# 0xPolygonZero/proof-protocol-decoder

Hardware: NVIDIA B200
Metric: mpt_nodes_keccak_hashed_per_sec (higher is better)
Workload: dtype u64

## Files before the change

### proof_protocol_decoder_b200/csrc/gpu_pre_image.cu

```cuda
#include "host_pipeline.h"

namespace ppd {

bool gpu_parse_enabled() {
#ifdef PPD_HOSTPROF
  return false;
#else
  return getenv("PPD_HOST_PARSE") == nullptr;
#endif
}

struct Carve {
  uint8_t* base;
  size_t off = 0;
  template <class T>
  T* take(size_t count) {
    off = (off + 255) & ~(size_t)255;
    T* r = reinterpret_cast<T*>(base + off);
    off += count * sizeof(T);
    return r;
  }
};

void upload_bytes(Lane* L, Job& J, uint8_t* dst, const uint8_t* src, size_t n) {
// ... 104 lines not shown
  const uint32_t n_ins = hr[PARSE_R_NINS];
  if (n_ins == 0 || n_ins > n) return false;
  if ((uint64_t)n_ins * 4 > (uint64_t)n + 256) return false;
  ParseTree T{};
  T.wit = B.wit, T.n = B.n, T.n_ins = n_ins, T.result = B.result;
  T.cnt_stride = ((size_t)n_ins + 1 + 3) & ~(size_t)3;
  uint32_t* ins_pos = nullptr;
  auto layout_b = [&](Carve& c) {
    const size_t n1 = (size_t)n_ins + 1;
    const size_t n_m1 = (n1 + 63) / 64, n_m2 = (n_m1 + 63) / 64, n_m3 = (n_m2 + 63) / 64;
    ins_pos = c.take<uint32_t>(n_ins);
    T.meta = c.take<uint32_t>(n_ins);
    T.knib = c.take<uint8_t>(n_ins);
    T.delta = c.take<uint32_t>(n1);
    T.hb = c.take<uint32_t>(n1);
    T.h16 = c.take<int16_t>(n1);
    T.m0 = c.take<int16_t>(8 * n_m1);
    T.m1 = c.take<int16_t>(n_m1);
    T.m2 = c.take<int16_t>(n_m2);
    T.m3 = c.take<int16_t>(n_m3);
    T.parent = c.take<uint32_t>(n_ins);
    T.info = c.take<uint32_t>(n_ins);
    T.aux0 = c.take<uint32_t>(n_ins);
    T.keyed = c.take<uint32_t>(n_ins);
    T.pending = c.take<uint32_t>(n_ins);
    T.lvlmax = c.take<uint32_t>(n_ins);
    T.cnt = c.take<uint32_t>(PARSE_N_CNT * T.cnt_stride);
    T.scn = c.take<uint32_t>(PARSE_N_CNT * T.cnt_stride);
    T.scan_tmp = c.take<uint32_t>(parse_scan_tmp_words(n1, PARSE_N_CNT));
  };
  {
    Carve sz{nullptr};
    layout_b(sz);
    L->d_pb.reserve(sz.off + 256);
    Carve c{L->d_pb.as<uint8_t>()};
    layout_b(c);
  }
  T.ins_pos = ins_pos;
  CUDA_OK(cudaEventRecord(L->ev0, st));
  launch_parse_scatter(B, ins_pos, st);
  L->stats.kernel_launches += 1 + launch_parse_tree(T, st);
  CUDA_OK(cudaGetLastError());
  CUDA_OK(cudaEventRecord(L->ev1, st));
  result_to_host();
  lane_sync(L);
  phase_ms();
  lap("p:B");
  trace_mark(L, "parse_b");
  if (hr[PARSE_R_FLAG] != 0 || hr[PARSE_R_HEIGHT] != 1) return false;
// ... 234 lines not shown
```

### proof_protocol_decoder_b200/csrc/ppd_kernels.h

```cpp
#pragma once
#include <cuda_runtime.h>

#include <cstdint>

#include "arena.h"
#include "txn_core.h"

namespace ppd {

void launch_keccak256_batch(const uint8_t* data, const uint64_t* offsets, uint32_t n, uint8_t* out, cudaStream_t st);
void launch_keccak256_ranges(const uint8_t* data, const uint64_t* begin_end, uint32_t n, uint8_t* out, cudaStream_t st);
void launch_hash_level(const ArenaView& A, const uint32_t* order, uint32_t begin, uint32_t end, cudaStream_t st);
static const uint32_t ORDER_MAX_BINS = 4096;
void launch_order_by_level_class(const NodeRec* nodes, const uint16_t* level, uint32_t n, uint32_t n_bins, uint16_t* keys, uint32_t* bins,
                                 uint32_t* order, cudaStream_t st, uint32_t first = 0, const uint32_t* n_dev = nullptr);

struct CopyBatch {
  static const uint32_t MAX = 16;
  void* dst[MAX];
  const void* src[MAX];
  unsigned long long bytes[MAX];
  uint32_t n = 0;
};
void launch_copy_segments(const CopyBatch& B, cudaStream_t st);
// ... 101 lines not shown
  uint32_t* exit1;
  uint16_t* step1;
  uint32_t* exit2;
  uint32_t* group_entry;
  uint32_t* tile_entry;
  uint32_t* bitmap;
  uint32_t* tile_count;
  uint32_t* tile_base;
  uint32_t* scan_tmp;
  uint32_t* result;
};
struct ParseTree {
  const uint8_t* wit;
  uint32_t n, n_ins;
  const uint32_t* ins_pos;
  uint32_t* meta;
  uint8_t* knib;
  uint32_t* delta;
  uint32_t* hb;
  int16_t *h16, *m0, *m1, *m2, *m3;
  uint32_t* parent;
  uint32_t* info;
  uint32_t* aux0;
  uint32_t* keyed;
  uint32_t *pending, *lvlmax;
  uint32_t *cnt, *scn;
  size_t cnt_stride;
  uint32_t* scan_tmp;
  uint32_t* result;
};
struct ParseEmit {
  ParseTree T;
  NodeRec* nodes;
  uint16_t* level;
  uint8_t *key_pool, *val_pool, *hash_pool;
  uint32_t* child_pool;
  AccountRec* accounts;
  uint32_t* acct_list;
  uint64_t* code_se;
  uint32_t* code_list;
  const uint8_t* code_digest;
  uint32_t n_keyed;
};
size_t parse_scan_tmp_words(size_t n, uint32_t K);
uint32_t launch_parse_bounds(const ParseBounds& B, cudaStream_t st);
void launch_parse_scatter(const ParseBounds& B, uint32_t* ins_pos, cudaStream_t st);
uint32_t launch_parse_tree(const ParseTree& T, cudaStream_t st);
void launch_parse_code_list(const ParseEmit& E, cudaStream_t st);
// ... 17 lines not shown
```

### proof_protocol_decoder_b200/csrc/ppd_parse.cu

```cuda
#include <cstdint>

#include "../../include/ppd_flat.h"
#include "../../include/ppd_status.h"
#include "arena.h"
#include "ppd_kernels.h"

namespace ppd {

namespace {

constexpr uint32_t TILE = PARSE_TILE;
constexpr uint32_t PERR = PARSE_ERR;
constexpr uint32_t NONE = 0xffffffffu;
constexpr uint32_t HASH_BASE = 0x80000000u;

__constant__ uint8_t C_EMPTY_TRIE_HASH[32] = {0x56, 0xe8, 0x1f, 0x17, 0x1b, 0xcc, 0x55, 0xa6, 0xff, 0x83, 0x45, 0xe6, 0x92, 0xc0, 0xf8, 0x6e,
                                              0x5b, 0x48, 0xe0, 0x1b, 0x99, 0x6c, 0xad, 0xc0, 0x01, 0x62, 0x2f, 0xb5, 0xe3, 0x63, 0xb4, 0x21};
__constant__ uint8_t C_EMPTY_CODE_HASH[32] = {0xc5, 0xd2, 0x46, 0x01, 0x86, 0xf7, 0x23, 0x3c, 0x92, 0x7e, 0x7d, 0xb2, 0xdc, 0xc7, 0x03, 0xc0,
                                              0xe5, 0x00, 0xb6, 0x53, 0xca, 0x82, 0x27, 0x3b, 0x7b, 0xfa, 0xd8, 0x04, 0x5d, 0x85, 0xa4, 0x70};

struct Ins {
  uint32_t op, next, flags, aux;
  uint32_t key_pos, key_len, val_pos, val_len;
  uint64_t nonce;
};

__device__ __forceinline__ bool cbor_head(const uint8_t* w, uint32_t n, uint32_t& pos, uint32_t& major, uint64_t& arg) {
  if (pos >= n) return false;
  uint32_t b = w[pos++];
  major = b >> 5;
  uint32_t ai = b & 31;
  if (ai < 24) {
    arg = ai;
    return true;
  }
  if (ai > 27) return false;
  uint32_t wd = 1u << (ai - 24);
  if (n - pos < wd) return false;
  arg = 0;
  for (uint32_t i = 0; i < wd; i++) arg = (arg << 8) | w[pos++];
  return true;
// ... 44 lines not shown
        if (!cbor_head(w, n, pos, major, arg) || major != 0) return PPD_ERR_INVALID_BYTES_FOR_TYPE;
        o.nonce = arg;
      }
      if (o.flags & 8) {
        if (!cbor_bytes(w, n, pos, o.val_pos, o.val_len) || o.val_len > 32) return PPD_ERR_INVALID_BYTE_VECTOR;
      }
      if (o.flags & 1) {
        if (!cbor_head(w, n, pos, major, arg) || major != 0) return PPD_ERR_INVALID_BYTES_FOR_TYPE;
      }
      break;
    case PPD_OP_EMPTY_ROOT:
      break;
    default:
      return PPD_ERR_INVALID_OPERATOR;
  }
  o.next = pos;
  return 0;
}
__device__ __forceinline__ uint32_t key_nibble_count(const uint8_t* __restrict__ w, uint32_t at, uint32_t len) {
  if (len == 0) return 0;
  if (len == 1) return 1;
  return 2 * (len - 1) - (__ldg(w + at) & 1u);
}
__device__ __forceinline__ void set_nib(uint8_t* pk, uint32_t d, uint32_t nib) { pk[d >> 1] |= (uint8_t)((d & 1) ? nib : (nib << 4)); }
__device__ __forceinline__ void put_key_nibbles(uint8_t* pk, uint32_t d, const uint8_t* __restrict__ w, uint32_t at, uint32_t len) {
  if (len == 0) return;
  if (len == 1) {
    set_nib(pk, d, __ldg(w + at) & 15u);
    return;
  }
  uint32_t cnt = 2 * (len - 1) - (__ldg(w + at) & 1u);
  for (uint32_t i = 0; i < cnt; i++) {
    uint32_t b = __ldg(w + at + 1 + (i >> 1));
    set_nib(pk, d + i, (i & 1) ? (b & 15u) : (b >> 4));
  }
}
__device__ __forceinline__ uint32_t nth_set_bit(uint32_t mask, uint32_t k) {
  for (uint32_t i = 0; i < k; i++) mask &= mask - 1;
  return mask ? (uint32_t)__ffs(mask) - 1 : 0u;
}

constexpr int TE_THREADS = 512;
constexpr uint32_t HALO = 128;

__device__ __forceinline__ void stage_tile(uint8_t* sb, const uint8_t* __restrict__ w, uint32_t n, uint32_t base, uint32_t tid, uint32_t nthreads) {
  const uint4* src = reinterpret_cast<const uint4*>(w + base);
  uint4* dst = reinterpret_cast<uint4*>(sb);
  const uint32_t avail = ((uint64_t)base + TILE + HALO <= (uint64_t)n + 48) ? (TILE + HALO) / 16 : (n + 48 - base) / 16;
  for (uint32_t k = tid; k < (TILE + HALO) / 16; k += nthreads) dst[k] = k < avail ? __ldg(src + k) : make_uint4(0, 0, 0, 0);
}

constexpr uint32_t TE_SMEM_BYTES = 4 * TILE + 4 * 2 * TILE + (TILE + HALO) + 16;

__global__ void __launch_bounds__(TE_THREADS, 4) tile_exit_kernel(const uint8_t* __restrict__ w, uint32_t n, uint32_t* __restrict__ exit1,
                                                                  uint16_t* __restrict__ step1) {
  extern __shared__ __align__(16) uint8_t te_smem[];
  uint32_t* nxt = reinterpret_cast<uint32_t*>(te_smem);
  uint16_t* step = reinterpret_cast<uint16_t*>(te_smem + 4 * TILE);
  uint16_t* active = step + TILE;
// ... 169 lines not shown
__global__ void __launch_bounds__(TILE / 32) ins_scatter_kernel(const uint32_t* __restrict__ bitmap, const uint32_t* __restrict__ tile_base,
                                                                uint32_t* __restrict__ ins_pos) {
  __shared__ uint32_t wsum[TILE / 32 / 32];
  const uint32_t t = blockIdx.x, tid = threadIdx.x;
  uint32_t word = bitmap[(size_t)t * (TILE / 32) + tid];
  uint32_t c = __popc(word), incl = c;
  for (int off = 1; off < 32; off <<= 1) {
    uint32_t x = __shfl_up_sync(0xffffffffu, incl, off);
    if ((tid & 31) >= (uint32_t)off) incl += x;
  }
  if ((tid & 31) == 31) wsum[tid >> 5] = incl;
  __syncthreads();
  uint32_t before = 0;
  for (uint32_t k = 0; k < (tid >> 5); k++) before += wsum[k];
  uint32_t at = tile_base[t] + before + incl - c;
  const uint32_t p0 = t * TILE + tid * 32;
  while (word) {
    uint32_t b = (uint32_t)__ffs(word) - 1;
    word &= word - 1;
    ins_pos[at++] = p0 + b;
  }
}

constexpr int MS_B = 256, MS_ITEMS = 4, MS_ELEMS = MS_B * MS_ITEMS;

__global__ void __launch_bounds__(MS_B) mscan_block_kernel(const uint32_t* __restrict__ in, uint32_t* __restrict__ out, uint32_t n, size_t stride,
                                                           uint32_t* __restrict__ block_sums, size_t sums_stride) {
  __shared__ uint32_t warp_sums[MS_B / 32];
  const uint32_t k = blockIdx.y;
  in += k * stride, out += k * stride;
  uint32_t base = blockIdx.x * MS_ELEMS + threadIdx.x * MS_ITEMS;
  uint32_t v[MS_ITEMS], sum = 0;
#pragma unroll
  for (int q = 0; q < MS_ITEMS; q++) {
    v[q] = base + q < n ? in[base + q] : 0u;
    sum += v[q];
  }
  uint32_t incl = sum;
  for (int off = 1; off < 32; off <<= 1) {
    uint32_t t = __shfl_up_sync(0xffffffffu, incl, off);
    if ((threadIdx.x & 31) >= (uint32_t)off) incl += t;
  }
  if ((threadIdx.x & 31) == 31) warp_sums[threadIdx.x >> 5] = incl;
  __syncthreads();
  if (threadIdx.x < 32) {
    uint32_t ws = threadIdx.x < MS_B / 32 ? warp_sums[threadIdx.x] : 0u, wi = ws;
    for (int off = 1; off < 32; off <<= 1) {
      uint32_t t = __shfl_up_sync(0xffffffffu, wi, off);
      if (threadIdx.x >= (uint32_t)off) wi += t;
    }
    if (threadIdx.x < MS_B / 32) warp_sums[threadIdx.x] = wi - ws;
    if (threadIdx.x == MS_B / 32 - 1 && block_sums) block_sums[k * sums_stride + blockIdx.x] = wi;
  }
  __syncthreads();
  uint32_t excl = incl - sum + warp_sums[threadIdx.x >> 5];
#pragma unroll
  for (int q = 0; q < MS_ITEMS; q++) {
    if (base + q < n) out[base + q] = excl;
    excl += v[q];
  }
}
__global__ void __launch_bounds__(MS_B) mscan_add_kernel(uint32_t* __restrict__ out, uint32_t n, size_t stride, const uint32_t* __restrict__ block_offsets,
                                                         size_t sums_stride) {
  const uint32_t k = blockIdx.y;
  out += k * stride;
  uint32_t add = block_offsets[k * sums_stride + blockIdx.x];
  uint32_t i = blockIdx.x * MS_ELEMS + threadIdx.x;
#pragma unroll
  for (int q = 0; q < MS_ITEMS; q++) {
    uint32_t j = i + q * MS_B;
    if (j < n) out[j] += add;
  }
}

uint32_t mscan(const uint32_t* in, uint32_t* out, uint32_t n, size_t stride, uint32_t K, uint32_t* tmp, cudaStream_t st) {
  if (!n) return 0;
  uint32_t nb = (n + MS_ELEMS - 1) / MS_ELEMS, launches = 1;
  size_t ss = (nb + 3) & ~(size_t)3;
  mscan_block_kernel<<<dim3(nb, K), MS_B, 0, st>>>(in, out, n, stride, nb > 1 ? tmp : nullptr, ss);
  if (nb > 1) {
    launches += mscan(tmp, tmp, nb, ss, K, tmp + K * ss, st);
    mscan_add_kernel<<<dim3(nb, K), MS_B, 0, st>>>(out, n, stride, tmp, ss);
    launches++;
  }
  return launches;
}

__device__ __forceinline__ uint32_t dw0(uint32_t kind, uint32_t nib_start, uint32_t nib_len) { return kind | (nib_start << 8) | (nib_len << 16); }
__device__ __forceinline__ void raise(uint32_t* result, uint32_t reason) { atomicCAS(result + PARSE_R_FLAG, 0u, reason); }

__device__ __forceinline__ uint32_t pops_of(uint32_t meta) {
  uint32_t op = meta & 7u;
  if (op == PPD_OP_EXTENSION) return 1;
  if (op == PPD_OP_BRANCH) return __popc(meta >> 16);
  if (op == PPD_OP_ACCOUNT_LEAF) return ((meta >> 8) & 1u) + ((meta >> 9) & 1u);
  return 0;
}

__device__ __forceinline__ void ins_info_one(const ParseTree& T, uint32_t i) {
  if (i == T.n_ins) {
    T.delta[i] = 0;
    return;
  }
  Ins o;
  uint32_t e = decode_ins(T.wit, T.n, T.ins_pos[i], o);
  if (e || o.op > 6) {
    raise(T.result, PARSE_WHY_DECODE);
    o.op = PPD_OP_EMPTY_ROOT, o.flags = 0, o.aux = 0, o.key_len = 0;
  }
  if (o.op == PPD_OP_BRANCH && (o.aux >> 16)) raise(T.result, PARSE_WHY_STACK);
  uint32_t meta = o.op | ((o.flags & 0xffu) << 8) | ((o.aux & 0xffffu) << 16);
  T.meta[i] = meta;
  uint32_t kn = key_nibble_count(T.wit, o.key_pos, o.key_len);
  T.knib[i] = (uint8_t)min(kn, 255u);
  uint32_t pops = pops_of(meta);
  T.delta[i] = 1u - pops;
  T.pending[i] = o.op == PPD_OP_ACCOUNT_LEAF ? ((o.flags >> 1) & 1u) : pops;
  T.lvlmax[i] = 0;
  T.aux0[i] = NONE;
}
__global__ void ins_info_kernel(ParseTree T) {
  uint32_t i = blockIdx.x * blockDim.x + threadIdx.x;
  if (i > T.n_ins) return;
  ins_info_one(T, i);
}

__global__ void heights_kernel(ParseTree T) {
  uint32_t i = blockIdx.x * blockDim.x + threadIdx.x;
  if (i > T.n_ins) return;
  if (i == T.n_ins) {
    T.h16[i] = INT16_MIN;
    T.result[PARSE_R_HEIGHT] = T.hb[i];
    return;
  }
  int32_t hb = (int32_t)T.hb[i];
  int32_t pops = (int32_t)pops_of(T.meta[i]);
  if (hb < pops) raise(T.result, PARSE_WHY_STACK);
  int32_t ha = hb + 1 - pops;
  if (ha > 30000 || ha < 1) {
    raise(T.result, PARSE_WHY_STACK);
    ha = ha < 1 ? 1 : 30000;
// ... 153 lines not shown
        decode_ins(T.wit, T.n, T.ins_pos[i], o);
        uint32_t vl = o.val_len, hl = 0;
        if (!(vl == 1 && __ldg(T.wit + o.val_pos) < 0x80)) hl = vl < 56 ? 1 : vl < 256 ? 2 : vl < 65536 ? 3 : vl < (1u << 24) ? 4 : 5;
        c_val = (hl + vl + 3) & ~3u;
      } else {
        if (in_storage) raise(T.result, PARSE_WHY_LEAF_KIND);
        c_acct = 1;
        uint32_t nonempty = 0;
        if (meta & (2u << 8)) {
          uint32_t sop = i ? (T.meta[i - 1] & 7u) : 7u;
          if (sop == PPD_OP_HASH) {
            const uint8_t* h = T.wit + T.ins_pos[i - 1] + 1;
            for (int k = 0; k < 32; k++) nonempty |= (uint32_t)(__ldg(h + k) != C_EMPTY_TRIE_HASH[k]);
          } else {
            nonempty = sop != PPD_OP_EMPTY_ROOT;
          }
        }
        c_node += nonempty;
        info |= nonempty << 17;
      }
    }
    info |= (min(d, 255u) << 8) | (in_storage << 16);
    T.info[i] = info;
  }
  T.cnt[PARSE_C_NODE * S + i] = c_node;
  T.cnt[PARSE_C_HASH * S + i] = c_hash;
  T.cnt[PARSE_C_KEY * S + i] = c_key;
  T.cnt[PARSE_C_VAL * S + i] = c_val;
  T.cnt[PARSE_C_CHILD * S + i] = c_child;
  T.cnt[PARSE_C_ACCT * S + i] = c_acct;
  T.cnt[PARSE_C_CODE * S + i] = c_code;
}
__global__ void __launch_bounds__(256) shape_kernel(ParseTree T) {
  __shared__ uint32_t n_here, base;
  const uint32_t i = blockIdx.x * blockDim.x + threadIdx.x;
  if (threadIdx.x == 0) n_here = 0;
  __syncthreads();
  bool keyed = false;
  if (i <= T.n_ins) {
    shape_one(T, i);
    if (i < T.n_ins) {
      const uint32_t op = T.meta[i] & 7u;
      keyed = op == PPD_OP_LEAF || op == PPD_OP_EXTENSION || op == PPD_OP_ACCOUNT_LEAF;
    }
  }
  const uint32_t at = keyed ? atomicAdd(&n_here, 1u) : 0u;
// ... 6 lines not shown
__global__ void totals_kernel(ParseTree T) {
  uint32_t k = threadIdx.x;
  if (k < PARSE_N_CNT) T.result[PARSE_R_TOTALS + k] = T.scn[k * T.cnt_stride + T.n_ins];
}

__device__ __forceinline__ uint32_t id_of(const ParseTree& T, uint32_t i) {
  uint32_t op = T.meta[i] & 7u;
  if (op == PPD_OP_HASH) return HASH_BASE + T.scn[PARSE_C_HASH * T.cnt_stride + i];
  if (op == PPD_OP_CODE || op == PPD_OP_EMPTY_ROOT) return NODE_EMPTY;
  return T.scn[PARSE_C_NODE * T.cnt_stride + i];
}

__global__ void code_list_kernel(ParseEmit E) {
  const ParseTree& T = E.T;
  uint32_t i = blockIdx.x * blockDim.x + threadIdx.x;
  if (i >= T.n_ins || (T.meta[i] & 7u) != PPD_OP_CODE) return;
  Ins o;
  decode_ins(T.wit, T.n, T.ins_pos[i], o);
  uint32_t c = T.scn[PARSE_C_CODE * T.cnt_stride + i];
  E.code_se[2 * c] = o.val_pos, E.code_se[2 * c + 1] = (uint64_t)o.val_pos + o.val_len;
  E.code_list[2 * c] = o.val_pos, E.code_list[2 * c + 1] = o.val_len;
}

__device__ __forceinline__ void copy_bytes(uint8_t* __restrict__ dst, const uint8_t* __restrict__ src, uint32_t n) {
  for (uint32_t k = 0; k < n; k++) dst[k] = __ldg(src + k);
}

__device__ __forceinline__ void emit_keyed(const ParseEmit& E, uint32_t i) {
  const ParseTree& T = E.T;
  const size_t S = T.cnt_stride;
  const uint32_t meta = T.meta[i], op = meta & 7u, info = T.info[i];
  const uint32_t pos = T.ins_pos[i];
  const uint32_t my_id = T.scn[PARSE_C_NODE * S + i];
  Ins o;
  decode_ins(T.wit, T.n, pos, o);
  const uint32_t d = (info >> 8) & 255u, kn = T.knib[i], nd = min(d + kn, 64u);
  uint8_t pk[36];
#pragma unroll
  for (int k = 0; k < 36; k++) pk[k] = 0;
  if (d + kn <= 64) put_key_nibbles(pk, d, T.wit, o.key_pos, o.key_len);
  {
    uint32_t cur = i;
    for (uint32_t guard = 0; guard < 4096; guard++) {
      uint32_t j = T.parent[cur];
      if (j >= T.n_ins) break;
      uint32_t pm = T.meta[j], pop = pm & 7u;
      uint32_t pd = (T.info[j] >> 8) & 255u;
      if (pop == PPD_OP_BRANCH) {
        if (pd < 64) set_nib(pk, pd, nth_set_bit(pm >> 16, T.info[cur] & 15u));
      } else if (pop == PPD_OP_EXTENSION) {
        Ins e;
        decode_ins(T.wit, T.n, T.ins_pos[j], e);
        if (pd + T.knib[j] <= 64) put_key_nibbles(pk, pd, T.wit, e.key_pos, e.key_len);
      } else {
        break;
      }
      cur = j;
    }
  }
  const uint32_t koff = T.scn[PARSE_C_KEY * S + i];
  {
    uint8_t* kd = E.key_pool + koff;
    uint32_t nb = (nd + 1) / 2;
    for (uint32_t k = 0; k < nb; k++) kd[k] = pk[k];
    kd[nb] = 0;
  }
  if (op == PPD_OP_EXTENSION) {
    E.nodes[my_id] = NodeRec{dw0(NK_EXT, d, kn), koff, i ? id_of(T, i - 1) : NODE_EMPTY, 0};
    return;
  }
  if (op == PPD_OP_LEAF) {
    uint32_t voff = T.scn[PARSE_C_VAL * S + i], vl = o.val_len, hl = 0;
    uint8_t* v = E.val_pool + voff;
    if (!(vl == 1 && __ldg(T.wit + o.val_pos) < 0x80)) {
      if (vl < 56) {
        v[hl++] = (uint8_t)(0x80 + vl);
      } else {
        uint32_t k = vl < 256 ? 1 : vl < 65536 ? 2 : vl < (1u << 24) ? 3 : 4;
        v[hl++] = (uint8_t)(0xb7 + k);
        for (uint32_t q = k; q-- > 0;) v[hl++] = (uint8_t)(vl >> (8 * q));
      }
    }
    copy_bytes(v + hl, T.wit + o.val_pos, vl);
    E.nodes[my_id] = NodeRec{dw0(NK_LEAF, d, kn), koff, voff, hl + vl};
    return;
  }
  const uint32_t a = T.scn[PARSE_C_ACCT * S + i];
  const uint32_t nonempty = (info >> 17) & 1u;
  uint32_t sroot = NODE_EMPTY, root_node = NODE_EMPTY;
  if (meta & (2u << 8)) sroot = i ? id_of(T, i - 1) : NODE_EMPTY;
  if (nonempty) {
    root_node = my_id + 1;
    E.nodes[root_node] = NodeRec{dw0(NK_ROOT, 0, 0), 0, sroot, 0};
  }
  {
    uint32_t* r = reinterpret_cast<uint32_t*>(E.accounts + a);
    uint8_t* rb = reinterpret_cast<uint8_t*>(r);
    for (int k = 0; k < 36; k++) r[k] = 0;
    for (int k = 0; k < 8; k++) rb[31 - k] = (uint8_t)(o.nonce >> (8 * k));
    if (meta & (8u << 8)) copy_bytes(rb + 32 + 32 - o.val_len, T.wit + o.val_pos, o.val_len);
    for (int k = 0; k < 32; k++) rb[64 + k] = C_EMPTY_TRIE_HASH[k];
    uint32_t code_idx = NONE;
    if (meta & (1u << 8)) {
      uint32_t ci = T.aux0[i];
      if (ci < T.n_ins) {
        if ((T.meta[ci] & 7u) == PPD_OP_CODE) {
          code_idx = T.scn[PARSE_C_CODE * S + ci];
          const uint8_t* dg = E.code_digest + 32ull * code_idx;
          for (int k = 0; k < 32; k++) rb[96 + k] = dg[k];
        } else {
          copy_bytes(rb + 96, T.wit + T.ins_pos[ci] + 1, 32);
        }
      }
    } else {
      for (int k = 0; k < 32; k++) rb[96 + k] = C_EMPTY_CODE_HASH[k];
    }
    r[32] = root_node;
    uint32_t* L = E.acct_list + 5ull * a;
    L[0] = my_id, L[1] = sroot, L[2] = root_node, L[3] = ((meta >> 9) & 1u) | (nonempty << 1), L[4] = code_idx;
  }
  E.nodes[my_id] = NodeRec{dw0(NK_LEAF_ACCOUNT, d, kn), koff, a, 0};
}

__global__ void __launch_bounds__(256) emit_kernel(ParseEmit E) {
  const ParseTree& T = E.T;
  const size_t S = T.cnt_stride;
  const uint32_t i = blockIdx.x * blockDim.x + threadIdx.x;
  if (i >= T.n_ins) return;
  const uint32_t meta = T.meta[i], op = meta & 7u, info = T.info[i];
  const uint32_t my_id = id_of(T, i);
  {
    uint32_t j = T.parent[i];
    if (j >= T.n_ins) T.result[PARSE_R_ROOT_ID] = my_id;
    if (j < T.n_ins && (T.meta[j] & 7u) == PPD_OP_BRANCH) E.child_pool[T.scn[PARSE_C_CHILD * S + j] + (info & 15u)] = my_id;
  }
  if (op == PPD_OP_HASH) {
    uint32_t* dst = reinterpret_cast<uint32_t*>(E.hash_pool + 32ull * (my_id - HASH_BASE));
    const uintptr_t a = reinterpret_cast<uintptr_t>(T.wit + T.ins_pos[i] + 1);
    const uint32_t* q = reinterpret_cast<const uint32_t*>(a & ~(uintptr_t)3);
    const uint32_t sh = (uint32_t)(a & 3) * 8;
// ... 15 lines not shown

__global__ void climb_kernel(ParseEmit E) {
  const ParseTree& T = E.T;
  uint32_t i = blockIdx.x * blockDim.x + threadIdx.x;
  if (i >= T.n_ins) return;
  const size_t S = T.cnt_stride;
  const uint32_t meta = T.meta[i], op = meta & 7u;
  const bool starter = op == PPD_OP_LEAF || op == PPD_OP_HASH || op == PPD_OP_EMPTY_ROOT || op == PPD_OP_CODE ||
                       (op == PPD_OP_ACCOUNT_LEAF && !(meta & (2u << 8)));
  if (!starter) return;
  if (op == PPD_OP_LEAF || op == PPD_OP_ACCOUNT_LEAF) E.level[T.scn[PARSE_C_NODE * S + i]] = 0;
  uint32_t cur = i, lv = 0;
  for (uint32_t guard = 0; guard < 4096; guard++) {
    uint32_t j = T.parent[cur];
    if (j >= T.n_ins) break;
    uint32_t pm = T.meta[j], pop = pm & 7u;
    uint32_t nid = T.scn[PARSE_C_NODE * S + j];
    if (pop == PPD_OP_ACCOUNT_LEAF) {
      if (((T.info[cur] >> 4) & 3u) != 2u) break;
      uint32_t nonempty = (T.info[j] >> 17) & 1u;
      if (nonempty) E.level[nid + 1] = (uint16_t)min(lv + 1, 65535u);
      lv = nonempty ? lv + 2 : 0;
    } else if (pop == PPD_OP_BRANCH || pop == PPD_OP_EXTENSION) {
      if (lv) {
        atomicMax(T.lvlmax + j, lv);
        __threadfence();
      }
      uint32_t old = atomicSub(T.pending + j, 1u);
      if (old != 1u) break;
      __threadfence();
      lv = atomicMax(T.lvlmax + j, 0u) + 1;
    } else {
      break;
    }
    E.level[nid] = (uint16_t)min(lv, 65535u);
    cur = j;
  }
}

inline uint32_t cdiv(uint64_t a, uint32_t b) { return (uint32_t)((a + b - 1) / b); }

}

size_t parse_scan_tmp_words(size_t n, uint32_t K) {
  size_t total = 0;
  while (n > 1) {
    n = (n + MS_ELEMS - 1) / MS_ELEMS;
    total += K * ((n + 3) & ~(size_t)3);
  }
  return total + 16;
}

uint32_t launch_parse_bounds(const ParseBounds& B, cudaStream_t st) {
  const uint32_t group_bytes = B.group_tiles * TILE;
  static const bool once = cudaFuncSetAttribute(tile_exit_kernel, cudaFuncAttributeMaxDynamicSharedMemorySize, (int)TE_SMEM_BYTES) == cudaSuccess;
  (void)once;
  tile_exit_kernel<<<B.n_tiles, TE_THREADS, TE_SMEM_BYTES, st>>>(B.wit, B.n, B.exit1, B.step1);
  group_exit_kernel<<<dim3(TILE / 256, B.n_groups), 256, 0, st>>>(B.exit1, B.n, group_bytes, B.exit2);
  cudaMemsetAsync(B.group_entry, 0xff, 4ull * B.n_groups, st);
  cudaMemsetAsync(B.tile_entry, 0xff, 4ull * B.n_tiles, st);
  top_chain_kernel<<<1, 32, 0, st>>>(B.exit1, B.exit2, B.n, group_bytes, B.group_entry, B.result);
  tile_entry_kernel<<<cdiv(B.n_groups, 64), 64, 0, st>>>(B.exit1, B.group_entry, B.n, B.n_groups, group_bytes, B.tile_entry);
  cudaMemsetAsync(B.bitmap, 0, (size_t)B.n_tiles * (TILE / 8), st);
  tile_mark_thin_kernel<<<cdiv(B.n_tiles, 128), 128, 0, st>>>(B.step1, B.n_tiles, B.tile_entry, B.bitmap, B.tile_count);
  cudaMemsetAsync(B.tile_count + B.n_tiles, 0, 4, st);
  uint32_t launches = 5 + mscan(B.tile_count, B.tile_base, B.n_tiles + 1, 0, 1, B.scan_tmp, st);
  cudaMemcpyAsync(B.result + PARSE_R_NINS, B.tile_base + B.n_tiles, 4, cudaMemcpyDeviceToDevice, st);
  return launches;
}

void launch_parse_scatter(const ParseBounds& B, uint32_t* ins_pos, cudaStream_t st) {
  ins_scatter_kernel<<<B.n_tiles, TILE / 32, 0, st>>>(B.bitmap, B.tile_base, ins_pos);
}

uint32_t launch_parse_tree(const ParseTree& T, cudaStream_t st) {
  const uint32_t n1 = T.n_ins + 1;
  ins_info_kernel<<<cdiv(n1, 256), 256, 0, st>>>(T);
  uint32_t launches = 8;
  launches += mscan(T.delta, T.hb, n1, 0, 1, T.scan_tmp, st);
  heights_kernel<<<cdiv(n1, 256), 256, 0, st>>>(T);
  const uint32_t n_m1 = cdiv(n1, 64), n_m2 = cdiv(n_m1, 64), n_m3 = cdiv(n_m2, 64);
  min8_64_i16_kernel<<<cdiv(n_m1, 128), 128, 0, st>>>(T.h16, n1, T.m0, T.m1, n_m1);
  min64_i16_kernel<<<cdiv(n_m2, 128), 128, 0, st>>>(T.m1, n_m1, T.m2, n_m2);
  min64_i16_kernel<<<cdiv(n_m3, 128), 128, 0, st>>>(T.m2, n_m2, T.m3, n_m3);
  link_kernel16<<<cdiv(T.n_ins, 256), 256, 0, st>>>(T);
  shape_kernel<<<cdiv(n1, 256), 256, 0, st>>>(T);
  launches += mscan(T.cnt, T.scn, n1, T.cnt_stride, PARSE_N_CNT, T.scan_tmp, st);
  totals_kernel<<<1, 32, 0, st>>>(T);
  return launches;
}

void launch_parse_code_list(const ParseEmit& E, cudaStream_t st) { code_list_kernel<<<cdiv(E.T.n_ins, 256), 256, 0, st>>>(E); }

void launch_parse_emit(const ParseEmit& E, cudaStream_t st) {
  emit_kernel<<<cdiv(E.T.n_ins, 256), 256, 0, st>>>(E);
  if (E.n_keyed) emit_keyed_kernel<<<cdiv(E.n_keyed, 128), 128, 0, st>>>(E);
  climb_kernel<<<cdiv(E.T.n_ins, 256), 256, 0, st>>>(E);
}

}
```

Before: 1.458 billion.

## Rework GPU witness parser: single-pass scan, packed walk records, word-wide emit

The recursive multi-launch block scan is replaced by a single-pass decoupled look-back scan with dynamic tile ids and vectorised loads and stores. The shape kernel now precomputes a packed per-node walk record, so emit_keyed climbs parents without re-decoding extension instructions, and key paths are built in registers with word-wide funnel shifts. Leaf values, account records and code hashes are written as 32-bit or 128-bit words instead of byte loops. The climb merges the pending counter and level max into one CAS word, dropping an array and several fences. This adds a kernel that spins on look-back state, and correctness now depends on pending counts fitting in 8 bits. A profiling script for per-kernel parse times is also added.

```diff
diff --git a/profiles/parse_kernel_times.py b/profiles/parse_kernel_times.py
--- /dev/null
+++ b/profiles/parse_kernel_times.py
@@ -0,0 +1,64 @@
+#!/usr/bin/env python3
+import os
+import re
+import subprocess
+import sys
+from collections import defaultdict
+
+ROOT = os.path.dirname(os.path.dirname(os.path.abspath(__file__)))
+sys.path.insert(0, ROOT)
+os.environ.setdefault("PPD_HOST_THREADS", "1")
+sys.dont_write_bytecode = True
+
+
+def short_name(name):
+    name = re.sub(r"ppd::\(anonymous namespace\)::", "", name)
+    name = re.sub(r"^void ", "", name)
+    return name.split("(")[0].split("<")[0]
+
+
+def main():
+    import torch
+    from torch.profiler import ProfilerActivity, profile
+
+    import bench
+    from proof_protocol_decoder_b200.lib import Context
+
+    replays = int(sys.argv[1]) if len(sys.argv) > 1 else 20
+    card = subprocess.run(["nvidia-smi", "--query-gpu=name,power.limit", "--format=csv,noheader", "-i", "0"],
+                          capture_output=True, text=True).stdout.strip()
+    flat = bench.c2_blocks([2], 1.0, 1)[0]
+    ctx = Context(0)
+    pinned = ctx.pinned_copy(flat)
+    with ctx.block_decode_view(pinned) as v:
+        _ = v.view[0]
+    st = ctx.stats()
+    assert st["witnesses_on_gpu"] == 1, "the block's witness did not take the GPU parser"
+    for _ in range(3):
+        ctx.replay_last(ctx.REPLAY_PARSE)
+    torch.cuda.synchronize()
+    with profile(activities=[ProfilerActivity.CUDA]) as prof:
+        for _ in range(replays):
+            ctx.replay_last(ctx.REPLAY_PARSE)
+        torch.cuda.synchronize()
+    us, count = defaultdict(float), defaultdict(int)
+    for e in prof.events():
+        if e.device_type != torch.autograd.DeviceType.CUDA:
+            continue
+        t = getattr(e, "device_time", None)
+        if t is None:
+            t = e.cuda_time
+        k = short_name(e.name)
+        us[k] += t
+        count[k] += 1
+    total = sum(us.values())
+    print(f"card: {card}")
+    print(f"block: config-2 seed 2, {st['witness_bytes']} witness bytes, {st['witness_instructions']} instructions; {replays} parse replays, one lane")
+    print(f"{'kernel':<28} {'us/replay':>10} {'launches':>9} {'share':>7}")
+    for k in sorted(us, key=us.get, reverse=True):
+        print(f"{k:<28} {us[k] / replays:10.1f} {count[k] / replays:9.1f} {100 * us[k] / total:6.1f}%")
+    print(f"{'total':<28} {total / replays:10.1f} {sum(count.values()) / replays:9.1f}")
+
+
+if __name__ == "__main__":
+    main()
diff --git a/proof_protocol_decoder_b200/csrc/gpu_pre_image.cu b/proof_protocol_decoder_b200/csrc/gpu_pre_image.cu
--- a/proof_protocol_decoder_b200/csrc/gpu_pre_image.cu
+++ b/proof_protocol_decoder_b200/csrc/gpu_pre_image.cu
@@ -150,9 +150,9 @@
     T.parent = c.take<uint32_t>(n_ins);
     T.info = c.take<uint32_t>(n_ins);
     T.aux0 = c.take<uint32_t>(n_ins);
+    T.walk = c.take<uint4>(n_ins);
     T.keyed = c.take<uint32_t>(n_ins);
     T.pending = c.take<uint32_t>(n_ins);
-    T.lvlmax = c.take<uint32_t>(n_ins);
     T.cnt = c.take<uint32_t>(PARSE_N_CNT * T.cnt_stride);
     T.scn = c.take<uint32_t>(PARSE_N_CNT * T.cnt_stride);
     T.scan_tmp = c.take<uint32_t>(parse_scan_tmp_words(n1, PARSE_N_CNT));
diff --git a/proof_protocol_decoder_b200/csrc/ppd_kernels.h b/proof_protocol_decoder_b200/csrc/ppd_kernels.h
--- a/proof_protocol_decoder_b200/csrc/ppd_kernels.h
+++ b/proof_protocol_decoder_b200/csrc/ppd_kernels.h
@@ -147,8 +147,9 @@
   uint32_t* parent;
   uint32_t* info;
   uint32_t* aux0;
+  uint4* walk;
   uint32_t* keyed;
-  uint32_t *pending, *lvlmax;
+  uint32_t* pending;
   uint32_t *cnt, *scn;
   size_t cnt_stride;
   uint32_t* scan_tmp;
diff --git a/proof_protocol_decoder_b200/csrc/ppd_parse.cu b/proof_protocol_decoder_b200/csrc/ppd_parse.cu
--- a/proof_protocol_decoder_b200/csrc/ppd_parse.cu
+++ b/proof_protocol_decoder_b200/csrc/ppd_parse.cu
@@ -14,9 +14,9 @@
 constexpr uint32_t NONE = 0xffffffffu;
 constexpr uint32_t HASH_BASE = 0x80000000u;
 
-__constant__ uint8_t C_EMPTY_TRIE_HASH[32] = {0x56, 0xe8, 0x1f, 0x17, 0x1b, 0xcc, 0x55, 0xa6, 0xff, 0x83, 0x45, 0xe6, 0x92, 0xc0, 0xf8, 0x6e,
+__constant__ __align__(16) uint8_t C_EMPTY_TRIE_HASH[32] = {0x56, 0xe8, 0x1f, 0x17, 0x1b, 0xcc, 0x55, 0xa6, 0xff, 0x83, 0x45, 0xe6, 0x92, 0xc0, 0xf8, 0x6e,
                                               0x5b, 0x48, 0xe0, 0x1b, 0x99, 0x6c, 0xad, 0xc0, 0x01, 0x62, 0x2f, 0xb5, 0xe3, 0x63, 0xb4, 0x21};
-__constant__ uint8_t C_EMPTY_CODE_HASH[32] = {0xc5, 0xd2, 0x46, 0x01, 0x86, 0xf7, 0x23, 0x3c, 0x92, 0x7e, 0x7d, 0xb2, 0xdc, 0xc7, 0x03, 0xc0,
+__constant__ __align__(16) uint8_t C_EMPTY_CODE_HASH[32] = {0xc5, 0xd2, 0x46, 0x01, 0x86, 0xf7, 0x23, 0x3c, 0x92, 0x7e, 0x7d, 0xb2, 0xdc, 0xc7, 0x03, 0xc0,
                                               0xe5, 0x00, 0xb6, 0x53, 0xca, 0x82, 0x27, 0x3b, 0x7b, 0xfa, 0xd8, 0x04, 0x5d, 0x85, 0xa4, 0x70};
 
 struct Ins {
@@ -107,19 +107,6 @@
   if (len == 1) return 1;
   return 2 * (len - 1) - (__ldg(w + at) & 1u);
 }
-__device__ __forceinline__ void set_nib(uint8_t* pk, uint32_t d, uint32_t nib) { pk[d >> 1] |= (uint8_t)((d & 1) ? nib : (nib << 4)); }
-__device__ __forceinline__ void put_key_nibbles(uint8_t* pk, uint32_t d, const uint8_t* __restrict__ w, uint32_t at, uint32_t len) {
-  if (len == 0) return;
-  if (len == 1) {
-    set_nib(pk, d, __ldg(w + at) & 15u);
-    return;
-  }
-  uint32_t cnt = 2 * (len - 1) - (__ldg(w + at) & 1u);
-  for (uint32_t i = 0; i < cnt; i++) {
-    uint32_t b = __ldg(w + at + 1 + (i >> 1));
-    set_nib(pk, d + i, (i & 1) ? (b & 15u) : (b >> 4));
-  }
-}
 __device__ __forceinline__ uint32_t nth_set_bit(uint32_t mask, uint32_t k) {
   for (uint32_t i = 0; i < k; i++) mask &= mask - 1;
   return mask ? (uint32_t)__ffs(mask) - 1 : 0u;
@@ -335,68 +322,105 @@
   }
 }
 
-constexpr int MS_B = 256, MS_ITEMS = 4, MS_ELEMS = MS_B * MS_ITEMS;
-
-__global__ void __launch_bounds__(MS_B) mscan_block_kernel(const uint32_t* __restrict__ in, uint32_t* __restrict__ out, uint32_t n, size_t stride,
-                                                           uint32_t* __restrict__ block_sums, size_t sums_stride) {
-  __shared__ uint32_t warp_sums[MS_B / 32];
-  const uint32_t k = blockIdx.y;
+constexpr int SC_B = 256, SC_ITEMS = 16, SC_ELEMS = SC_B * SC_ITEMS;
+constexpr unsigned long long SC_AGG = 1ull << 32, SC_PFX = 2ull << 32;
+
+__device__ __forceinline__ unsigned long long ld_relaxed(const unsigned long long* p) {
+  unsigned long long v;
+  asm volatile("ld.relaxed.gpu.global.u64 %0, [%1];" : "=l"(v) : "l"(p) : "memory");
+  return v;
+}
+__device__ __forceinline__ void st_relaxed(unsigned long long* p, unsigned long long v) {
+  asm volatile("st.relaxed.gpu.global.u64 [%0], %1;" ::"l"(p), "l"(v) : "memory");
+}
+
+__global__ void __launch_bounds__(SC_B) scan_kernel(const uint32_t* __restrict__ in, uint32_t* __restrict__ out, uint32_t n, size_t stride, uint32_t nb,
+                                                    unsigned long long* __restrict__ state) {
+  __shared__ uint32_t warp_sums[SC_B / 32], s_tile, s_prefix;
+  const uint32_t lane = threadIdx.x & 31;
+  if (threadIdx.x == 0) s_tile = atomicAdd(reinterpret_cast<unsigned int*>(state), 1u);
+  __syncthreads();
+  const uint32_t id = s_tile, k = id / nb, t = id - k * nb;
   in += k * stride, out += k * stride;
-  uint32_t base = blockIdx.x * MS_ELEMS + threadIdx.x * MS_ITEMS;
-  uint32_t v[MS_ITEMS], sum = 0;
-#pragma unroll
-  for (int q = 0; q < MS_ITEMS; q++) {
-    v[q] = base + q < n ? in[base + q] : 0u;
-    sum += v[q];
-  }
+  unsigned long long* tiles = state + 1 + (size_t)k * nb;
+  const uint32_t base = t * SC_ELEMS + threadIdx.x * SC_ITEMS;
+  uint32_t v[SC_ITEMS], sum = 0;
+  if (base + SC_ITEMS <= n) {
+#pragma unroll
+    for (int q = 0; q < SC_ITEMS / 4; q++) {
+      const uint4 a = reinterpret_cast<const uint4*>(in + base)[q];
+      v[4 * q] = a.x, v[4 * q + 1] = a.y, v[4 * q + 2] = a.z, v[4 * q + 3] = a.w;
+    }
+  } else {
+#pragma unroll
+    for (int q = 0; q < SC_ITEMS; q++) v[q] = base + q < n ? in[base + q] : 0u;
+  }
+#pragma unroll
+  for (int q = 0; q < SC_ITEMS; q++) sum += v[q];
   uint32_t incl = sum;
+#pragma unroll
   for (int off = 1; off < 32; off <<= 1) {
-    uint32_t t = __shfl_up_sync(0xffffffffu, incl, off);
-    if ((threadIdx.x & 31) >= (uint32_t)off) incl += t;
-  }
-  if ((threadIdx.x & 31) == 31) warp_sums[threadIdx.x >> 5] = incl;
+    const uint32_t x = __shfl_up_sync(0xffffffffu, incl, off);
+    if (lane >= (uint32_t)off) incl += x;
+  }
+  if (lane == 31) warp_sums[threadIdx.x >> 5] = incl;
   __syncthreads();
   if (threadIdx.x < 32) {
-    uint32_t ws = threadIdx.x < MS_B / 32 ? warp_sums[threadIdx.x] : 0u, wi = ws;
+    const uint32_t ws = lane < SC_B / 32 ? warp_sums[lane] : 0u;
+    uint32_t wi = ws;
+#pragma unroll
     for (int off = 1; off < 32; off <<= 1) {
-      uint32_t t = __shfl_up_sync(0xffffffffu, wi, off);
-      if (threadIdx.x >= (uint32_t)off) wi += t;
-    }
-    if (threadIdx.x < MS_B / 32) warp_sums[threadIdx.x] = wi - ws;
-    if (threadIdx.x == MS_B / 32 - 1 && block_sums) block_sums[k * sums_stride + blockIdx.x] = wi;
+      const uint32_t x = __shfl_up_sync(0xffffffffu, wi, off);
+      if (lane >= (uint32_t)off) wi += x;
+    }
+    if (lane < SC_B / 32) warp_sums[lane] = wi - ws;
+    const uint32_t agg = __shfl_sync(0xffffffffu, wi, 31);
+    uint32_t prefix = 0;
+    if (t == 0) {
+      if (lane == 0) st_relaxed(tiles, SC_PFX | agg);
+    } else {
+      if (lane == 0) st_relaxed(tiles + t, SC_AGG | agg);
+      for (int32_t end = (int32_t)t;; end -= 32) {
+        const int32_t j = end - 1 - (int32_t)lane;
+        unsigned long long s = SC_PFX;
+        if (j >= 0) {
+          do s = ld_relaxed(tiles + j);
+          while ((s >> 32) == 0);
+        }
+        const uint32_t pfx = __ballot_sync(0xffffffffu, (s & SC_PFX) != 0);
+        const uint32_t last = pfx ? (uint32_t)__ffs(pfx) - 1 : 31u;
+        uint32_t x = lane <= last ? (uint32_t)s : 0u;
+#pragma unroll
+        for (int off = 16; off; off >>= 1) x += __shfl_xor_sync(0xffffffffu, x, off);
+        prefix += x;
+        if (pfx) break;
+      }
+      if (lane == 0) st_relaxed(tiles + t, SC_PFX | (prefix + agg));
+    }
+    if (lane == 0) s_prefix = prefix;
   }
   __syncthreads();
-  uint32_t excl = incl - sum + warp_sums[threadIdx.x >> 5];
-#pragma unroll
-  for (int q = 0; q < MS_ITEMS; q++) {
-    if (base + q < n) out[base + q] = excl;
-    excl += v[q];
-  }
-}
-__global__ void __launch_bounds__(MS_B) mscan_add_kernel(uint32_t* __restrict__ out, uint32_t n, size_t stride, const uint32_t* __restrict__ block_offsets,
-                                                         size_t sums_stride) {
-  const uint32_t k = blockIdx.y;
-  out += k * stride;
-  uint32_t add = block_offsets[k * sums_stride + blockIdx.x];
-  uint32_t i = blockIdx.x * MS_ELEMS + threadIdx.x;
-#pragma unroll
-  for (int q = 0; q < MS_ITEMS; q++) {
-    uint32_t j = i + q * MS_B;
-    if (j < n) out[j] += add;
-  }
-}
-
-uint32_t mscan(const uint32_t* in, uint32_t* out, uint32_t n, size_t stride, uint32_t K, uint32_t* tmp, cudaStream_t st) {
-  if (!n) return 0;
-  uint32_t nb = (n + MS_ELEMS - 1) / MS_ELEMS, launches = 1;
-  size_t ss = (nb + 3) & ~(size_t)3;
-  mscan_block_kernel<<<dim3(nb, K), MS_B, 0, st>>>(in, out, n, stride, nb > 1 ? tmp : nullptr, ss);
-  if (nb > 1) {
-    launches += mscan(tmp, tmp, nb, ss, K, tmp + K * ss, st);
-    mscan_add_kernel<<<dim3(nb, K), MS_B, 0, st>>>(out, n, stride, tmp, ss);
-    launches++;
-  }
-  return launches;
+  uint32_t excl = incl - sum + warp_sums[threadIdx.x >> 5] + s_prefix;
+  uint32_t o[SC_ITEMS];
+#pragma unroll
+  for (int q = 0; q < SC_ITEMS; q++) o[q] = excl, excl += v[q];
+  if (base + SC_ITEMS <= n) {
+#pragma unroll
+    for (int q = 0; q < SC_ITEMS / 4; q++) reinterpret_cast<uint4*>(out + base)[q] = make_uint4(o[4 * q], o[4 * q + 1], o[4 * q + 2], o[4 * q + 3]);
+  } else {
+#pragma unroll
+    for (int q = 0; q < SC_ITEMS; q++)
+      if (base + q < n) out[base + q] = o[q];
+  }
+}
+
+uint32_t scan_tiles(size_t n) { return (uint32_t)((n + SC_ELEMS - 1) / SC_ELEMS); }
+
+void scan(const uint32_t* in, uint32_t* out, uint32_t n, size_t stride, uint32_t K, uint32_t* tmp, cudaStream_t st) {
+  const uint32_t nb = scan_tiles(n);
+  unsigned long long* state = reinterpret_cast<unsigned long long*>(tmp);
+  cudaMemsetAsync(state, 0, 8ull * (1 + (size_t)K * nb), st);
+  scan_kernel<<<K * nb, SC_B, 0, st>>>(in, out, n, stride, nb, state);
 }
 
 __device__ __forceinline__ uint32_t dw0(uint32_t kind, uint32_t nib_start, uint32_t nib_len) { return kind | (nib_start << 8) | (nib_len << 16); }
@@ -429,7 +453,6 @@
   uint32_t pops = pops_of(meta);
   T.delta[i] = 1u - pops;
   T.pending[i] = o.op == PPD_OP_ACCOUNT_LEAF ? ((o.flags >> 1) & 1u) : pops;
-  T.lvlmax[i] = 0;
   T.aux0[i] = NONE;
 }
 __global__ void ins_info_kernel(ParseTree T) {
@@ -629,6 +652,18 @@
     }
     info |= (min(d, 255u) << 8) | (in_storage << 16);
     T.info[i] = info;
+    if (op != PPD_OP_LEAF) {
+      uint32_t y = op | ((info & 15u) << 4) | (min(d, 255u) << 8), key_at = 0;
+      if (op == PPD_OP_BRANCH) {
+        y |= meta & 0xffff0000u;
+      } else if (op == PPD_OP_EXTENSION) {
+        Ins e;
+        decode_ins(T.wit, T.n, T.ins_pos[i], e);
+        y |= (e.key_len == 1 ? 8u : 0u) | (min(kn, 255u) << 16);
+        key_at = e.key_len == 1 ? e.key_pos : e.key_pos + 1;
+      }
+      T.walk[i] = make_uint4(T.parent[i], y, key_at, 0u);
+    }
   }
   T.cnt[PARSE_C_NODE * S + i] = c_node;
   T.cnt[PARSE_C_HASH * S + i] = c_hash;
@@ -681,67 +716,138 @@
   E.code_list[2 * c] = o.val_pos, E.code_list[2 * c + 1] = o.val_len;
 }
 
-__device__ __forceinline__ void copy_bytes(uint8_t* __restrict__ dst, const uint8_t* __restrict__ src, uint32_t n) {
-  for (uint32_t k = 0; k < n; k++) dst[k] = __ldg(src + k);
+__device__ __forceinline__ void path_set_nib(uint32_t (&pk)[8], uint32_t d, uint32_t nib) {
+  const uint32_t v = nib << (28 - 4 * (d & 7u)), q = d >> 3;
+#pragma unroll
+  for (uint32_t w = 0; w < 8; w++) pk[w] |= q == w ? v : 0u;
+}
+__device__ __forceinline__ void load32(const uint8_t* p, uint32_t (&x)[8]) {
+  const uintptr_t a = reinterpret_cast<uintptr_t>(p);
+  const uint32_t* q = reinterpret_cast<const uint32_t*>(a & ~(uintptr_t)3);
+  const uint32_t sh = (uint32_t)(a & 3) * 8;
+  uint32_t y[9];
+#pragma unroll
+  for (int c = 0; c < 9; c++) y[c] = __ldg(q + c);
+#pragma unroll
+  for (int c = 0; c < 8; c++) x[c] = __funnelshift_r(y[c], y[c + 1], sh);
+}
+__device__ __forceinline__ void path_put(uint32_t (&pk)[8], uint32_t d, const uint8_t* src, uint32_t cnt) {
+  uint32_t x[8];
+  load32(src, x);
+#pragma unroll
+  for (int w = 0; w < 8; w++) {
+    const int r = (int)cnt - 8 * w;
+    x[w] = __byte_perm(x[w], 0u, 0x0123) & (r >= 8 ? 0xffffffffu : r <= 0 ? 0u : 0xffffffffu << (32 - 4 * r));
+  }
+  const uint32_t sh = 4 * (d & 7u), q = d >> 3;
+#pragma unroll
+  for (int w = 7; w >= 0; w--) x[w] = __funnelshift_r(x[w], w ? x[w - 1] : 0u, sh);
+#pragma unroll
+  for (int w = 7; w >= 0; w--) x[w] = (q & 1u) ? (w >= 1 ? x[w - 1] : 0u) : x[w];
+#pragma unroll
+  for (int w = 7; w >= 0; w--) x[w] = (q & 2u) ? (w >= 2 ? x[w - 2] : 0u) : x[w];
+#pragma unroll
+  for (int w = 7; w >= 0; w--) x[w] = (q & 4u) ? (w >= 4 ? x[w - 4] : 0u) : x[w];
+#pragma unroll
+  for (int w = 0; w < 8; w++) pk[w] |= x[w];
+}
+__device__ __forceinline__ void path_put_key(uint32_t (&pk)[8], uint32_t d, const uint8_t* __restrict__ w, uint32_t at, uint32_t len, uint32_t cnt) {
+  if (len == 1) path_set_nib(pk, d, __ldg(w + at) & 15u);
+  if (len >= 2) path_put(pk, d, w + at + 1, cnt);
+}
+__device__ __forceinline__ void load_be256(const uint8_t* p, uint32_t len, uint32_t (&x)[8]) {
+  load32(p, x);
+#pragma unroll
+  for (int w = 0; w < 8; w++) {
+    const int r = (int)len - 4 * w;
+    x[w] &= r >= 4 ? 0xffffffffu : r <= 0 ? 0u : (1u << (8 * r)) - 1u;
+  }
+  const uint32_t up = 32 - len, sh = 8 * (up & 3u), q = up >> 2;
+#pragma unroll
+  for (int w = 7; w >= 0; w--) x[w] = __funnelshift_l(w ? x[w - 1] : 0u, x[w], sh);
+#pragma unroll
+  for (int w = 7; w >= 0; w--) x[w] = (q & 1u) ? (w >= 1 ? x[w - 1] : 0u) : x[w];
+#pragma unroll
+  for (int w = 7; w >= 0; w--) x[w] = (q & 2u) ? (w >= 2 ? x[w - 2] : 0u) : x[w];
+#pragma unroll
+  for (int w = 7; w >= 0; w--) x[w] = (q & 4u) ? (w >= 4 ? x[w - 4] : 0u) : x[w];
 }
 
 __device__ __forceinline__ void emit_keyed(const ParseEmit& E, uint32_t i) {
   const ParseTree& T = E.T;
   const size_t S = T.cnt_stride;
   const uint32_t meta = T.meta[i], op = meta & 7u, info = T.info[i];
-  const uint32_t pos = T.ins_pos[i];
   const uint32_t my_id = T.scn[PARSE_C_NODE * S + i];
   Ins o;
-  decode_ins(T.wit, T.n, pos, o);
+  decode_ins(T.wit, T.n, T.ins_pos[i], o);
   const uint32_t d = (info >> 8) & 255u, kn = T.knib[i], nd = min(d + kn, 64u);
-  uint8_t pk[36];
-#pragma unroll
-  for (int k = 0; k < 36; k++) pk[k] = 0;
-  if (d + kn <= 64) put_key_nibbles(pk, d, T.wit, o.key_pos, o.key_len);
+  uint32_t pk[8] = {0, 0, 0, 0, 0, 0, 0, 0};
+  if (d + kn <= 64) path_put_key(pk, d, T.wit, o.key_pos, o.key_len, kn);
   {
-    uint32_t cur = i;
-    for (uint32_t guard = 0; guard < 4096; guard++) {
-      uint32_t j = T.parent[cur];
-      if (j >= T.n_ins) break;
-      uint32_t pm = T.meta[j], pop = pm & 7u;
-      uint32_t pd = (T.info[j] >> 8) & 255u;
+    uint32_t slot = info & 15u, j = T.parent[i];
+    for (uint32_t guard = 0; guard < 4096 && j < T.n_ins; guard++) {
+      const uint4 r = __ldg(T.walk + j);
+      const uint32_t pop = r.y & 7u, pd = (r.y >> 8) & 255u;
       if (pop == PPD_OP_BRANCH) {
-        if (pd < 64) set_nib(pk, pd, nth_set_bit(pm >> 16, T.info[cur] & 15u));
+        if (pd < 64) path_set_nib(pk, pd, nth_set_bit(r.y >> 16, slot));
       } else if (pop == PPD_OP_EXTENSION) {
-        Ins e;
-        decode_ins(T.wit, T.n, T.ins_pos[j], e);
-        if (pd + T.knib[j] <= 64) put_key_nibbles(pk, pd, T.wit, e.key_pos, e.key_len);
+        const uint32_t pkn = r.y >> 16;
+        if (pd + pkn <= 64) {
+          if (r.y & 8u)
+            path_set_nib(pk, pd, __ldg(T.wit + r.z) & 15u);
+          else
+            path_put(pk, pd, T.wit + r.z, pkn);
+        }
       } else {
         break;
       }
-      cur = j;
+      slot = (r.y >> 4) & 15u, j = r.x;
     }
   }
   const uint32_t koff = T.scn[PARSE_C_KEY * S + i];
   {
     uint8_t* kd = E.key_pool + koff;
-    uint32_t nb = (nd + 1) / 2;
-    for (uint32_t k = 0; k < nb; k++) kd[k] = pk[k];
-    kd[nb] = 0;
+    const uint32_t nb = (nd + 1) / 2;
+#pragma unroll
+    for (uint32_t k = 0; k < 32; k++)
+      if (k <= nb) kd[k] = k < nb ? (uint8_t)(pk[k >> 2] >> (24 - 8 * (k & 3u))) : 0u;
+    if (nb == 32) kd[32] = 0;
   }
   if (op == PPD_OP_EXTENSION) {
     E.nodes[my_id] = NodeRec{dw0(NK_EXT, d, kn), koff, i ? id_of(T, i - 1) : NODE_EMPTY, 0};
     return;
   }
   if (op == PPD_OP_LEAF) {
-    uint32_t voff = T.scn[PARSE_C_VAL * S + i], vl = o.val_len, hl = 0;
-    uint8_t* v = E.val_pool + voff;
+    const uint32_t voff = T.scn[PARSE_C_VAL * S + i], vl = o.val_len;
+    uint32_t hl = 0;
+    uint64_t hdr = 0;
     if (!(vl == 1 && __ldg(T.wit + o.val_pos) < 0x80)) {
       if (vl < 56) {
-        v[hl++] = (uint8_t)(0x80 + vl);
+        hdr = 0x80 + vl, hl = 1;
       } else {
-        uint32_t k = vl < 256 ? 1 : vl < 65536 ? 2 : vl < (1u << 24) ? 3 : 4;
-        v[hl++] = (uint8_t)(0xb7 + k);
-        for (uint32_t q = k; q-- > 0;) v[hl++] = (uint8_t)(vl >> (8 * q));
-      }
-    }
-    copy_bytes(v + hl, T.wit + o.val_pos, vl);
-    E.nodes[my_id] = NodeRec{dw0(NK_LEAF, d, kn), koff, voff, hl + vl};
+        const uint32_t k = vl < 256 ? 1 : vl < 65536 ? 2 : vl < (1u << 24) ? 3 : 4;
+        hdr = 0xb7 + k, hl = k + 1;
+        for (uint32_t m = 1; m <= k; m++) hdr |= (uint64_t)((vl >> (8 * (k - m))) & 0xffu) << (8 * m);
+      }
+    }
+    const uint32_t total = hl + vl, nw = (total + 3) / 4;
+    uint32_t* v = reinterpret_cast<uint32_t*>(E.val_pool + voff);
+    const uintptr_t src = reinterpret_cast<uintptr_t>(T.wit + o.val_pos - hl);
+    const uint32_t* q = reinterpret_cast<const uint32_t*>(src & ~(uintptr_t)3);
+    const uint32_t sh = (uint32_t)(src & 3) * 8;
+    uint32_t lo = __ldg(q);
+    for (uint32_t k = 0; k < nw; k++) {
+      const uint32_t hi = __ldg(q + k + 1);
+      uint32_t x = __funnelshift_r(lo, hi, sh);
+      lo = hi;
+      if (4 * k < hl) {
+        const uint32_t nh = min(hl - 4 * k, 4u), m = nh == 4 ? 0xffffffffu : (1u << (8 * nh)) - 1u;
+        x = (x & ~m) | ((uint32_t)(hdr >> (32 * k)) & m);
+      }
+      if (4 * k + 4 > total) x &= (1u << (8 * (total - 4 * k))) - 1u;
+      v[k] = x;
+    }
+    E.nodes[my_id] = NodeRec{dw0(NK_LEAF, d, kn), koff, voff, total};
     return;
   }
   const uint32_t a = T.scn[PARSE_C_ACCT * S + i];
@@ -753,28 +859,33 @@
     E.nodes[root_node] = NodeRec{dw0(NK_ROOT, 0, 0), 0, sroot, 0};
   }
   {
-    uint32_t* r = reinterpret_cast<uint32_t*>(E.accounts + a);
-    uint8_t* rb = reinterpret_cast<uint8_t*>(r);
-    for (int k = 0; k < 36; k++) r[k] = 0;
-    for (int k = 0; k < 8; k++) rb[31 - k] = (uint8_t)(o.nonce >> (8 * k));
-    if (meta & (8u << 8)) copy_bytes(rb + 32 + 32 - o.val_len, T.wit + o.val_pos, o.val_len);
-    for (int k = 0; k < 32; k++) rb[64 + k] = C_EMPTY_TRIE_HASH[k];
+    uint4* r = reinterpret_cast<uint4*>(E.accounts + a);
+    const uint4 z = make_uint4(0, 0, 0, 0);
+    r[0] = z;
+    r[1] = make_uint4(0, 0, __byte_perm((uint32_t)(o.nonce >> 32), 0u, 0x0123), __byte_perm((uint32_t)o.nonce, 0u, 0x0123));
+    uint32_t b[8] = {0, 0, 0, 0, 0, 0, 0, 0};
+    if (meta & (8u << 8)) load_be256(T.wit + o.val_pos, o.val_len, b);
+    r[2] = make_uint4(b[0], b[1], b[2], b[3]), r[3] = make_uint4(b[4], b[5], b[6], b[7]);
+    r[4] = reinterpret_cast<const uint4*>(C_EMPTY_TRIE_HASH)[0], r[5] = reinterpret_cast<const uint4*>(C_EMPTY_TRIE_HASH)[1];
     uint32_t code_idx = NONE;
+    uint4 c0 = reinterpret_cast<const uint4*>(C_EMPTY_CODE_HASH)[0], c1 = reinterpret_cast<const uint4*>(C_EMPTY_CODE_HASH)[1];
     if (meta & (1u << 8)) {
-      uint32_t ci = T.aux0[i];
+      c0 = c1 = z;
+      const uint32_t ci = T.aux0[i];
       if (ci < T.n_ins) {
         if ((T.meta[ci] & 7u) == PPD_OP_CODE) {
           code_idx = T.scn[PARSE_C_CODE * S + ci];
-          const uint8_t* dg = E.code_digest + 32ull * code_idx;
-          for (int k = 0; k < 32; k++) rb[96 + k] = dg[k];
+          const uint4* dg = reinterpret_cast<const uint4*>(E.code_digest + 32ull * code_idx);
+          c0 = dg[0], c1 = dg[1];
         } else {
-          copy_bytes(rb + 96, T.wit + T.ins_pos[ci] + 1, 32);
+          uint32_t h[8];
+          load32(T.wit + T.ins_pos[ci] + 1, h);
+          c0 = make_uint4(h[0], h[1], h[2], h[3]), c1 = make_uint4(h[4], h[5], h[6], h[7]);
         }
       }
-    } else {
-      for (int k = 0; k < 32; k++) rb[96 + k] = C_EMPTY_CODE_HASH[k];
-    }
-    r[32] = root_node;
+    }
+    r[6] = c0, r[7] = c1;
+    r[8] = make_uint4(root_node, 0, 0, 0);
     uint32_t* L = E.acct_list + 5ull * a;
     L[0] = my_id, L[1] = sroot, L[2] = root_node, L[3] = ((meta >> 9) & 1u) | (nonempty << 1), L[4] = code_idx;
   }
@@ -836,14 +947,19 @@
       if (nonempty) E.level[nid + 1] = (uint16_t)min(lv + 1, 65535u);
       lv = nonempty ? lv + 2 : 0;
     } else if (pop == PPD_OP_BRANCH || pop == PPD_OP_EXTENSION) {
+      uint32_t old;
       if (lv) {
-        atomicMax(T.lvlmax + j, lv);
-        __threadfence();
-      }
-      uint32_t old = atomicSub(T.pending + j, 1u);
-      if (old != 1u) break;
-      __threadfence();
-      lv = atomicMax(T.lvlmax + j, 0u) + 1;
+        old = *reinterpret_cast<volatile uint32_t*>(T.pending + j);
+        for (;;) {
+          const uint32_t seen = atomicCAS(T.pending + j, old, (max(old >> 8, lv) << 8) | ((old & 255u) - 1u));
+          if (seen == old) break;
+          old = seen;
+        }
+      } else {
+        old = atomicSub(T.pending + j, 1u);
+      }
+      if ((old & 255u) != 1u) break;
+      lv = max(old >> 8, lv) + 1;
     } else {
       break;
     }
@@ -856,14 +972,7 @@
 
 }
 
-size_t parse_scan_tmp_words(size_t n, uint32_t K) {
-  size_t total = 0;
-  while (n > 1) {
-    n = (n + MS_ELEMS - 1) / MS_ELEMS;
-    total += K * ((n + 3) & ~(size_t)3);
-  }
-  return total + 16;
-}
+size_t parse_scan_tmp_words(size_t n, uint32_t K) { return 2 * (1 + (size_t)K * scan_tiles(n)); }
 
 uint32_t launch_parse_bounds(const ParseBounds& B, cudaStream_t st) {
   const uint32_t group_bytes = B.group_tiles * TILE;
@@ -878,9 +987,9 @@
   cudaMemsetAsync(B.bitmap, 0, (size_t)B.n_tiles * (TILE / 8), st);
   tile_mark_thin_kernel<<<cdiv(B.n_tiles, 128), 128, 0, st>>>(B.step1, B.n_tiles, B.tile_entry, B.bitmap, B.tile_count);
   cudaMemsetAsync(B.tile_count + B.n_tiles, 0, 4, st);
-  uint32_t launches = 5 + mscan(B.tile_count, B.tile_base, B.n_tiles + 1, 0, 1, B.scan_tmp, st);
+  scan(B.tile_count, B.tile_base, B.n_tiles + 1, 0, 1, B.scan_tmp, st);
   cudaMemcpyAsync(B.result + PARSE_R_NINS, B.tile_base + B.n_tiles, 4, cudaMemcpyDeviceToDevice, st);
-  return launches;
+  return 6;
 }
 
 void launch_parse_scatter(const ParseBounds& B, uint32_t* ins_pos, cudaStream_t st) {
@@ -890,8 +999,7 @@
 uint32_t launch_parse_tree(const ParseTree& T, cudaStream_t st) {
   const uint32_t n1 = T.n_ins + 1;
   ins_info_kernel<<<cdiv(n1, 256), 256, 0, st>>>(T);
-  uint32_t launches = 8;
-  launches += mscan(T.delta, T.hb, n1, 0, 1, T.scan_tmp, st);
+  scan(T.delta, T.hb, n1, 0, 1, T.scan_tmp, st);
   heights_kernel<<<cdiv(n1, 256), 256, 0, st>>>(T);
   const uint32_t n_m1 = cdiv(n1, 64), n_m2 = cdiv(n_m1, 64), n_m3 = cdiv(n_m2, 64);
   min8_64_i16_kernel<<<cdiv(n_m1, 128), 128, 0, st>>>(T.h16, n1, T.m0, T.m1, n_m1);
@@ -899,9 +1007,9 @@
   min64_i16_kernel<<<cdiv(n_m3, 128), 128, 0, st>>>(T.m2, n_m2, T.m3, n_m3);
   link_kernel16<<<cdiv(T.n_ins, 256), 256, 0, st>>>(T);
   shape_kernel<<<cdiv(n1, 256), 256, 0, st>>>(T);
-  launches += mscan(T.cnt, T.scn, n1, T.cnt_stride, PARSE_N_CNT, T.scan_tmp, st);
+  scan(T.cnt, T.scn, n1, T.cnt_stride, PARSE_N_CNT, T.scan_tmp, st);
   totals_kernel<<<1, 32, 0, st>>>(T);
-  return launches;
+  return 10;
 }
 
 void launch_parse_code_list(const ParseEmit& E, cudaStream_t st) { code_list_kernel<<<cdiv(E.T.n_ins, 256), 256, 0, st>>>(E); }
```

New measurement: 1.460 billion, median of 6. No clear change (+0.1%).
